# apple/ml-neuman

Hardware: NVIDIA H100
Metric: Mrays/sec @128+128 samples (higher is better)
Workload: dtype f16 operands x f32 accumulate (wgmma); f32 elsewhere

## Files before the change

neuman_b200/csrc/mlp_tc.cu:

```cuda
#include "nm_internal.cuh"
#include "nm_pe.cuh"
#include "tc_common.cuh"
#include <string.h>
#define TC_MAX_SLABS 64
struct TcPlan {
  uint32_t slab_off[TC_STEPS][6];
  uint32_t slab_bytes[TC_STEPS];
  uint32_t image_bytes;
  uint32_t lin_off[TC_MAX_SLABS + 1];
};

__host__ __device__ constexpr int tc_steps(bool v) { return v ? TC_STEPS : 9; }
__host__ __device__ constexpr int step_nkb(int s, bool v = true, bool t = false) {
  return s == 0 ? (t ? 2 : 1) : (s == 10 ? 2 : (!v && s == 8 ? 4 : (t && s == 5 ? 6 : 5)));
}
__host__ __device__ constexpr bool kb_is_bias(int s, int kb, bool v = true) {
  return kb == 4 && s != 5 && s != 9 && s >= 1 && (v ? s <= 8 : s <= 7);
}
__host__ __device__ constexpr bool kb_is_time(int s, int kb, bool t) { return t && ((s == 0 && kb == 1) || (s == 5 && kb == 5)); }
__host__ __device__ constexpr int step_N(int s, bool v = true) { return s <= 7 || (v && s == 8) ? 256 : (v && s == 9 ? 128 : 16); }
__host__ __device__ constexpr bool kb_is_dir(int s, int kb, bool v = true) { return v && s == 9 && kb == 4; }
__host__ __device__ constexpr int tc_slabs_per_tile(bool v = true, bool t = false) {
  int n = 0;
  for (int s = 0; s < tc_steps(v); ++s) n += step_nkb(s, v, t);
  return n;
}
static_assert(tc_slabs_per_tile(true, true) <= TC_MAX_SLABS && tc_slabs_per_tile(true) <= TC_MAX_SLABS, "slab table too small");

template <bool kTrain, bool kView>
struct TcCfg {
  static constexpr int THREADS = 256;
  static constexpr int NSLOT = kTrain || kView ? 4 : 6;
  static constexpr int OFF_POS = kTrain ? 4 * TC_KB_BYTES : 0;
  static constexpr int OFF_DIR = OFF_POS + TC_KB_BYTES;
  static constexpr int WG_BYTES = OFF_DIR + TC_KB_BYTES;
  static constexpr int OFF_RING = 2 * WG_BYTES;
  static constexpr int OFF_BAR = OFF_RING + NSLOT * TC_SLAB_BYTES;
  static constexpr int OFF_CONST = OFF_BAR + 16 * NSLOT;
  static constexpr int SMEM_USED = OFF_CONST + 4 * TC_CONST_FLOATS;
  static constexpr int SMEM_BYTES = SMEM_USED + 1024;
};
static_assert(TcCfg<false, false>::SMEM_BYTES <= 232448 && TcCfg<false, true>::SMEM_BYTES <= 232448 &&
              TcCfg<true, false>::SMEM_BYTES <= 232448 && TcCfg<true, true>::SMEM_BYTES <= 232448,
              "shared memory of the forward kernel exceeds 227 KB");

#define TC_CONST_ALPHA 0
#define TC_CONST_OUT 256

struct TcParams {
  const uint8_t* wimg;
  TcPlan plan;
  NmMlpInput in;
  NmPeSpec pos_pe, dir_pe;
  float* raw;
  const float* consts;
  long long n_tiles;
  int32_t* range_flag;
  int range_phase;
  __half* st_x;
  __half* st_f;
  __half* st_v;
  uint32_t* st_m;
  CUtensorMap map_x, map_f, map_v;
};

__device__ __forceinline__ void sincos_cycles(float f, float& s, float& c) {
  f = f - rintf(f);
  const float a = f * 6.283185307179586f;
  s = __sinf(a);
  c = __cosf(a);
}

__device__ __forceinline__ void encode_f16(const NmPeSpec& pe, const float x[3], uint32_t (&out)[32], int nq) {
  float ch[64];
#pragma unroll
  for (int i = 0; i < 64; ++i) ch[i] = 0.f;
// ... 94 lines not shown
    }
    const uint32_t pA = pack2<RELU>(x0, x1), pB = pack2<RELU>(y0, y1);
    if (SMEM) {
      uint8_t* blk = act + (j >> 3) * TC_KB_BYTES;
      *reinterpret_cast<uint32_t*>(blk + swz_off(rA, c)) = pA;
      *reinterpret_cast<uint32_t*>(blk + swz_off(rB, c)) = pB;
    } else {
      a[2 * j] = pA;
      a[2 * j + 1] = pB;
    }
    if (track) { track_range<RELU>(rng, pA); track_range<RELU>(rng, pB); }
    if (SIGNS) {
      const __half2 zero2 = __float2half2_rn(0.f);
      const uint32_t mA = __hgt2_mask(*reinterpret_cast<const __half2*>(&pA), zero2);
      const uint32_t mB = __hgt2_mask(*reinterpret_cast<const __half2*>(&pB), zero2);
      const int bit = 16 * ((j >> 1) & 1) + 4 * (j & 1) + q;
      wA[j >> 2] |= ((mA & 1u) << bit) | ((mA >> 16 & 1u) << (bit + 8));
      wB[j >> 2] |= ((mB & 1u) << bit) | ((mB >> 16 & 1u) << (bit + 8));
    }
  }
}

__device__ __forceinline__ void quad_or(uint32_t (&w)[8]) {
#pragma unroll
  for (int i = 0; i < 8; ++i) {
    w[i] |= __shfl_xor_sync(0xffffffffu, w[i], 1);
    w[i] |= __shfl_xor_sync(0xffffffffu, w[i], 2);
  }
}

template <bool kTrain, bool kView, bool kTime = false>
__device__ __forceinline__ void mlp_tc_body(const TcParams& P) {
  static_assert(!kTime || kView, "NeRF-T nets are view-dependent");
  using C = TcCfg<kTrain, kView>;
  constexpr int SLABS = tc_slabs_per_tile(kView, kTime);
  constexpr int STEPS = tc_steps(kView);
  constexpr int LAST = STEPS - 1;
  extern __shared__ uint8_t smem_dyn[];
  const uint32_t pad = (1024 - (smem_u32(smem_dyn) & 1023)) & 1023;
  uint8_t* smem = smem_dyn + pad;
  const uint32_t sbase = smem_u32(smem);
  const int wg = threadIdx.x >> 7, wtid = threadIdx.x & 127;
  const int lane = threadIdx.x & 31, q = lane & 3;
  const int rA = 16 * (wtid >> 5) + (lane >> 2);
  uint8_t* wbuf = smem + wg * C::WG_BYTES;
  const uint32_t wbase = sbase + wg * C::WG_BYTES;
  float* s_const = reinterpret_cast<float*>(smem + C::OFF_CONST);
  const TcRing<C::NSLOT> R{sbase + C::OFF_RING, sbase + C::OFF_BAR};

  for (int i = threadIdx.x; i < TC_CONST_FLOATS; i += C::THREADS) s_const[i] = __ldg(P.consts + i);
  const long long my_tiles = blockIdx.x < P.n_tiles ? (P.n_tiles - 1 - blockIdx.x) / gridDim.x + 1 : 0;
  const uint32_t total = (uint32_t)(my_tiles * SLABS);
  auto fill = [&](uint32_t qq) {
    const uint32_t j = qq % SLABS, off = P.plan.lin_off[j], bytes = P.plan.lin_off[j + 1] - off;
    mbar_arrive_expect_tx(R.full(qq), bytes);
    bulk_g2s(R.slot(qq), P.wimg + off, bytes, R.full(qq));
  };
  if (threadIdx.x == 0) R.init(total, fill);
  __syncthreads();

  const float4 ob = *reinterpret_cast<const float4*>(s_const + TC_CONST_OUT);
  float d[128];
  float d16[8];
  uint32_t a[64];
  uint32_t rng = 0;
  uint32_t qbase = 0;
  const long long rperiod = my_tiles < 64 ? my_tiles : 64;
  for (long long it = 0; it < my_tiles; ++it) {
    const long long tile = blockIdx.x + it * gridDim.x;
    const long long row0 = tile * 128 + wg * TC_WG_ROWS;
    const bool track = !kView || (it % rperiod) == (P.range_phase % rperiod);
    {
      const int r = wtid & 63;
      const int group = P.in.group;
      long long g0 = 0;
      uint32_t g0r = 0;
      if (group > 0) { g0 = tile * 128 / group; g0r = (uint32_t)(tile * 128 - g0 * group); }
      const uint32_t off = wg * TC_WG_ROWS + r;
      const long long g = group > 0 ? g0 + (g0r + off) / (uint32_t)group : row0 + r;
      float p[3] = {0.f, 0.f, 0.f}, v[3] = {0.f, 0.f, 0.f};
      float t = 0.f;
      if (row0 + r < P.in.n) {
        nm_fetch_sample_at<kTime ? 4 : 3>(P.in, row0 + r, g, p, v);
        if (kTime) t = nm_fetch_time(P.in, row0 + r);
      }
      if (!kTrain && it > 0) wg_sync(wg);
      uint32_t e[32];
      if (wtid < 64) {
        encode_f16(P.pos_pe, p, e, 30);
        store_row_swizzled(wbuf + C::OFF_POS, r, e, 8);
      } else if (kView) {
        encode_f16(P.dir_pe, v, e, 12);
        if (kTime) encode_time_f16(P.pos_pe, t, e);
        store_row_swizzled(wbuf + C::OFF_DIR, r, e, kTime ? 8 : 4);
      }
      if (track && (kView || wtid < 64)) { track_range<false>(rng, e[0]); track_range<false>(rng, e[1]); }
      if (kTime && track && wtid >= 64) track_range<false>(rng, e[16]);
      fence_async_smem();
      wg_sync(wg);
    }
    float alpha[2] = {0.f, 0.f};
#pragma unroll (kTrain ? 1 : STEPS)
    for (int s = 0; s < STEPS; ++s) {
      const int nkb = step_nkb(s, kView, kTime);
      const bool wide = s <= (kView ? 8 : 7), views = kView && s == 9;
      wgmma_fence();
      int kb = 0;
      auto kblock = [&](auto&& issue) {
        const uint32_t qq = qbase + kb;
        R.wait_full(qq);
        issue(gmma_desc_k(R.slot(qq)), kb == 0);
        wgmma_commit();
        if (kb > 0) { wgmma_wait<1>(); R.release(qq - 1, total, fill); }
        ++kb;
      };
      auto smem_kblock = [&](uint32_t a_addr, int k0, int k1) {
        kblock([&](uint64_t b_desc, bool first) {
          const uint64_t a_desc = gmma_desc_k(a_addr);
          for (int k = k0; k < k1; ++k) {
            const uint32_t acc = !first || k > k0;
            if (wide) wgmma_n256(d, a_desc + 2 * k, b_desc + 2 * k, acc);
            else if (views) wgmma_n128(d, a_desc + 2 * k, b_desc + 2 * k, acc);
            else wgmma_n16(d16, a_desc + 2 * k, b_desc + 2 * k, acc);
          }
        });
      };
      if (s == 0 || s == 5) smem_kblock(wbase + C::OFF_POS, 0, 4);
      if (s > 0) {
        const int nact = kView && s == LAST ? 2 : 4;
#pragma unroll
        for (int j = 0; j < 4; ++j) {
          if (j < nact) {
            if constexpr (kTrain) smem_kblock(wbase + j * TC_KB_BYTES, 0, 4);
            else kblock([&](uint64_t b_desc, bool first) {
#pragma unroll
              for (int k = 0; k < 4; ++k) {
                const uint32_t* f = a + 16 * j + 4 * k;
                const uint32_t acc = !first || k > 0;
                if (wide) wgmma_n256_rs(d, f[0], f[1], f[2], f[3], b_desc + 2 * k, acc);
                else if (views) wgmma_n128_rs(d, f[0], f[1], f[2], f[3], b_desc + 2 * k, acc);
                else wgmma_n16_rs(d16, f[0], f[1], f[2], f[3], b_desc + 2 * k, acc);
              }
            });
          }
        }
      }
      if (kb < nkb) {
        if (kb_is_bias(s, kb, kView)) smem_kblock(wbase + C::OFF_POS, 3, 4);
        else if (kb_is_dir(s, kb, kView)) smem_kblock(wbase + C::OFF_DIR, 0, 2);
        else smem_kblock(wbase + C::OFF_DIR, 2, 4);
      }
      wgmma_wait<0>();
      wgmma_fence_regs(d);
      wgmma_fence_regs(d16);
      R.release(qbase + nkb - 1, total, fill);
      qbase += nkb;
      if (s < LAST) {
        if (kTrain) {
          if (wtid == 0) tma_store_wait_read();
          wg_sync(wg);
        }
        uint32_t wA[8] = {0, 0, 0, 0, 0, 0, 0, 0}, wB[8] = {0, 0, 0, 0, 0, 0, 0, 0};
        const float* s_walpha = s_const + TC_CONST_ALPHA;
        if (s == 7) fwd_epi<256, true, kView, kTrain, kTrain>(d, a, wbuf, rA, q, s_walpha, alpha, wA, wB, track, rng);
        else if (kView && s == 8) fwd_epi<256, false, false, false, kTrain>(d, a, wbuf, rA, q, s_walpha, alpha, wA, wB, track, rng);
        else if (s == 9) fwd_epi<128, true, false, kTrain, kTrain>(d, a, wbuf, rA, q, s_walpha, alpha, wA, wB, track, rng);
        else fwd_epi<256, true, false, kTrain, kTrain>(d, a, wbuf, rA, q, s_walpha, alpha, wA, wB, track, rng);
        if (kTrain) {
          fence_async_smem();
          wg_sync(wg);
          if (wtid == 0) {
            if (!kView || s < 8) tma_store_rows(&P.map_x, wbase, 0, 4, row0, s);
            else if (s == 8) tma_store_rows(&P.map_f, wbase, 0, 4, row0, 0);
            else tma_store_rows(&P.map_v, wbase, 0, 2, row0, 0);
          }
          if (!kView || s != 8) {
            quad_or(wA);
            quad_or(wB);
            const long long iA = row0 + rA, iB = iA + 8;
            if (!kView || s < 8) {
              uint32_t* m = P.st_m + (size_t)s * P.in.n * 8;
              if (iA < P.in.n) reinterpret_cast<uint2*>(m + iA * 8)[q] = make_uint2(wA[2 * q], wA[2 * q + 1]);
              if (iB < P.in.n) reinterpret_cast<uint2*>(m + iB * 8)[q] = make_uint2(wB[2 * q], wB[2 * q + 1]);
            } else {
              uint32_t* m = P.st_m + (size_t)8 * P.in.n * 8;
              if (iA < P.in.n) m[iA * 8 + q] = wA[q];
              if (iB < P.in.n) m[iB * 8 + q] = wB[q];
            }
          }
// ... 28 lines not shown
}

template <bool kTrain>
__global__ void __launch_bounds__(TcCfg<kTrain, true>::THREADS, 1) k_mlp_tc(const __grid_constant__ TcParams P) {
  mlp_tc_body<kTrain, true>(P);
}
template <bool kTrain>
__global__ void __launch_bounds__(TcCfg<kTrain, false>::THREADS, 1) k_mlp_tc_noview(const __grid_constant__ TcParams P) {
  mlp_tc_body<kTrain, false>(P);
}
template <bool kTrain>
__global__ void __launch_bounds__(TcCfg<kTrain, true>::THREADS, 1) k_mlp_tc_nerft(const __grid_constant__ TcParams P) {
  mlp_tc_body<kTrain, true, true>(P);
}

struct PackSrc {
  const float* w[8]; const float* feat; const float* views; const float* rgb;
  const float* b[8]; const float* feat_b; const float* views_b;
  const float* out_t;
};

__device__ __forceinline__ int nerft_col(int kk, bool time) {
  if (time) {
    if (kk == 32) return 3;
    if (kk < 33 || kk > 52) return -1;
    const int k = (kk - 33) >> 1;
    return ((kk - 33) & 1) ? 11 + 8 * k : 7 + 8 * k;
  }
  if (kk < 3) return kk;
  const int i = kk - 3, k = i / 6, r = i - 6 * k;
  return r < 3 ? 4 + 8 * k + r : 8 + 8 * k + (r - 3);
}

__device__ __forceinline__ float src_weight(const PackSrc& S, int s, int n, int kb, int kk, bool view, bool time) {
  if (!view && s == 8) return n < 4 ? S.out_t[(size_t)(kb * 64 + kk) * 4 + n] : 0.f;
  if (kb_is_bias(s, kb, view)) {
    if (kk != 63) return 0.f;
    return s == 8 ? S.feat_b[n] : S.b[s][n];
  }
  if (time && (s == 0 || s == 5)) {
    const int ld = s == 0 ? NM_POS_PE_T : NM_POS_PE_T + 256;
    const float* w = S.w[s] + (size_t)n * ld;
    if (kb_is_time(s, kb, true)) {
      const int c = nerft_col(kk, true);
      return c < 0 ? 0.f : w[c];
    }
    if (kb == 0) return kk < NM_POS_PE ? w[nerft_col(kk, false)] : S.b[s][n];
    return w[NM_POS_PE_T + (kb - 1) * 64 + kk];
  }
  if (s == 0) return kk < NM_POS_PE ? S.w[0][(size_t)n * NM_POS_PE + kk] : S.b[0][n];
  if (s >= 1 && s <= 7 && s != 5) return S.w[s][(size_t)n * 256 + kb * 64 + kk];
  if (s == 5) {
    const int ld = NM_POS_PE + 256;
    if (kb == 0) return kk < NM_POS_PE ? S.w[5][(size_t)n * ld + kk] : S.b[5][n];
    return S.w[5][(size_t)n * ld + NM_POS_PE + (kb - 1) * 64 + kk];
  }
  if (s == 8) return S.feat[(size_t)n * 256 + kb * 64 + kk];
  if (s == 9) {
    const int ld = 256 + NM_DIR_PE;
    if (kb < 4) return S.views[(size_t)n * ld + kb * 64 + kk];
    return kk < NM_DIR_PE ? S.views[(size_t)n * ld + 256 + kk] : (kk == NM_DIR_PE ? S.views_b[n] : 0.f);
  }
  return n < 3 ? S.rgb[(size_t)n * 128 + kb * 64 + kk] : 0.f;
}

__global__ void k_tc_pack(PackSrc S, TcPlan plan, bool view, bool time, __half* __restrict__ out) {
  const size_t e = (size_t)blockIdx.x * blockDim.x + threadIdx.x;
  if (e * 2 >= plan.image_bytes) return;
  const uint32_t byte = (uint32_t)(e * 2);
  int s = 0, kb = 0;
  for (int ss = 0; ss < tc_steps(view); ++ss)
    for (int k = 0; k < step_nkb(ss, view, time); ++k)
      if (byte >= plan.slab_off[ss][k]) { s = ss; kb = k; }
  const uint32_t in_slab = byte - plan.slab_off[s][kb];
  const int n = in_slab >> 7;
  const int chunk_phys = (in_slab & 127) >> 4;
  const int chunk = chunk_phys ^ (n & 7);
  const int kk = chunk * 8 + ((in_slab & 15) >> 1);
  out[e] = __float2half_rn(src_weight(S, s, n, kb, kk, view, time));
}

__global__ void k_tc_consts(const float* rgb_b, const float* alpha_w, const float* alpha_b, float* __restrict__ out) {
  const int i = threadIdx.x;
  out[TC_CONST_ALPHA + i] = alpha_w[i];
  if (i < TC_CONST_FLOATS - TC_CONST_OUT) out[TC_CONST_OUT + i] = i < 3 ? rgb_b[i] : (i == 3 ? alpha_b[0] : 0.f);
}
__global__ void k_tc_consts_noview(const float* out_b, float* __restrict__ out) {
  const int i = threadIdx.x;
  out[TC_CONST_ALPHA + i] = 0.f;
  if (i < TC_CONST_FLOATS - TC_CONST_OUT) out[TC_CONST_OUT + i] = i < 4 ? out_b[i] : 0.f;
}

__global__ void k_encode_f16(NmPeSpec pe, int which, const float* __restrict__ x, long long group, long long n,
                             __half* __restrict__ out) {
  const long long i = (long long)blockIdx.x * blockDim.x + threadIdx.x;
  if (i >= n) return;
  const long long xi = group > 0 ? i / group : i;
  const float xv[3] = {x[3 * xi], x[3 * xi + 1], x[3 * xi + 2]};
  uint32_t e[32];
  encode_f16(pe, xv, e, which == 0 ? 30 : 12);
  if (which == 0) {
    e[31] |= 0x3C000000u;
    uint4* dst = reinterpret_cast<uint4*>(out + (size_t)i * 64);
#pragma unroll
    for (int j = 0; j < 8; ++j) dst[j] = make_uint4(e[4 * j], e[4 * j + 1], e[4 * j + 2], e[4 * j + 3]);
  } else {
    e[13] |= 0x3C000000u;
    uint4* dst = reinterpret_cast<uint4*>(out + (size_t)i * 32);
#pragma unroll
    for (int j = 0; j < 4; ++j) dst[j] = make_uint4(e[4 * j], e[4 * j + 1], e[4 * j + 2], e[4 * j + 3]);
  }
}
// ... 8 lines not shown
  for (int c = 0; c < 96; ++c) ch[c] = 0.f;
#pragma unroll
  for (int d = 0; d < 4; ++d) ch[d] = x[4 * xi + d];
#pragma unroll
  for (int k = 0; k < 10; ++k) {
    const float fh = __ldg(pe.table + 2 * k), fl = __ldg(pe.table + 2 * k + 1);
#pragma unroll
    for (int d = 0; d < 4; ++d) {
      const float v = ch[d];
      const float pr = v * fh;
      const float low = fmaf(v, fl, fmaf(v, fh, -pr));
      sincos_cycles((pr - rintf(pr)) + low, ch[4 + 8 * k + d], ch[8 + 8 * k + d]);
    }
  }
  ch[NM_POS_PE_T] = 1.f;
  uint4* dst = reinterpret_cast<uint4*>(out + (size_t)i * 96);
#pragma unroll
  for (int j = 0; j < 12; ++j)
    dst[j] = make_uint4(pack_f16x2(ch[8 * j], ch[8 * j + 1], false), pack_f16x2(ch[8 * j + 2], ch[8 * j + 3], false),
                        pack_f16x2(ch[8 * j + 4], ch[8 * j + 5], false), pack_f16x2(ch[8 * j + 6], ch[8 * j + 7], false));
}

int nm_tc_encode(nm_ctx* ctx, const NmNet& net, int which, const float* x, int64_t group, int64_t n, __half* out, cudaStream_t st) {
  NmPeSpec pe = which == 0 ? NmPeSpec{net.desc.pos_pe_kind, net.desc.pos_n_freqs, net.f32 + net.o_pos_cyc}
                           : NmPeSpec{net.desc.dir_pe_kind, net.desc.dir_n_freqs, net.f32 + net.o_dir_cyc};
  if (which == 0 && net.kind == NM_NET_NERFT)
    k_encode_f16_nerft<<<(unsigned)((n + 127) / 128), 128, 0, st>>>(pe, x, group, n, out);
  else
    k_encode_f16<<<(unsigned)((n + 127) / 128), 128, 0, st>>>(pe, which, x, group, n, out);
  NM_CHECK_LAUNCH(ctx);
  return NM_OK;
}

static TcPlan make_plan(bool view, bool time) {
  TcPlan p{};
  uint32_t off = 0;
  int j = 0;
  for (int s = 0; s < tc_steps(view); ++s) {
    p.slab_bytes[s] = (uint32_t)step_N(s, view) * 128u;
    for (int kb = 0; kb < step_nkb(s, view, time); ++kb) {
      p.slab_off[s][kb] = p.lin_off[j++] = off;
      off += p.slab_bytes[s];
    }
  }
  p.lin_off[j] = p.image_bytes = off;
  return p;
}

int nm_tc_pack(nm_ctx* ctx, NmNet& net, cudaStream_t st) {
  const bool view = net.kind != NM_NET_NOVIEW, time = net.kind == NM_NET_NERFT;
  TcPlan plan = make_plan(view, time);
  const size_t halfs = plan.image_bytes / 2;
  if (!net.f16 || net.f16_halfs != halfs) {
    if (net.f16) { NM_CHECK_CUDA(ctx, cudaDeviceSynchronize()); NM_CHECK_CUDA(ctx, cudaFree(net.f16)); net.f16 = nullptr; }
    NM_CHECK_CUDA(ctx, cudaMalloc(&net.f16, halfs * sizeof(__half)));
    net.f16_halfs = halfs;
  }
  if (!net.tc_bias) NM_CHECK_CUDA(ctx, cudaMalloc(&net.tc_bias, TC_CONST_FLOATS * sizeof(float)));
  const nm_nerf_desc& d = net.desc;
  PackSrc S;
  for (int l = 0; l < 8; ++l) S.w[l] = d.pts_w[l];
  S.feat = d.feature_w; S.views = d.views_w; S.rgb = d.rgb_w;
  for (int l = 0; l < 8; ++l) S.b[l] = d.pts_b[l];
  S.feat_b = d.feature_b; S.views_b = d.views_b;
  S.out_t = net.f32 + net.o_out_w;
  k_tc_pack<<<(unsigned)((halfs + 255) / 256), 256, 0, st>>>(S, plan, view, time, net.f16);
  NM_CHECK_LAUNCH(ctx);
  if (view) k_tc_consts<<<1, 256, 0, st>>>(d.rgb_b, d.alpha_w, d.alpha_b, net.tc_bias);
  else k_tc_consts_noview<<<1, 256, 0, st>>>(net.f32 + net.o_out_b, net.tc_bias);
  NM_CHECK_LAUNCH(ctx);
  return NM_OK;
}

template <bool kTrain, bool kView, bool kTime = false>
static int launch_tc(nm_ctx* ctx, const TcParams& P, cudaStream_t st) {
  void (*kernel)(const TcParams);
  if constexpr (kTime) kernel = k_mlp_tc_nerft<kTrain>;
  else kernel = kView ? k_mlp_tc<kTrain> : k_mlp_tc_noview<kTrain>;
  using C = TcCfg<kTrain, kView>;
  NM_SET_SMEM_ONCE(ctx, kernel, C::SMEM_BYTES);
  long long ctas = ctx->sm_count;
  if (P.n_tiles < ctas) ctas = P.n_tiles > 0 ? P.n_tiles : 1;
  kernel<<<(unsigned)ctas, C::THREADS, C::SMEM_BYTES, st>>>(P);
  NM_CHECK_LAUNCH(ctx);
  return NM_OK;
}

int nm_tc_forward(nm_ctx* ctx, NmNet& net, const float* pts, const float* views, const float* origins,
                  const float* dirs, const float* z, int64_t n, int32_t group, float t, float* raw, cudaStream_t st,
                  const NmTrainStash* stash) {
  if (!net.f16 || !net.tc_bias) NM_FAIL(ctx, NM_ERR_STATE, "nm_tc_forward: weights not packed");
  const bool view = net.kind != NM_NET_NOVIEW, time = net.kind == NM_NET_NERFT;
  TcParams P;
  P.wimg = reinterpret_cast<const uint8_t*>(net.f16);
  P.plan = make_plan(view, time);
  P.in = NmMlpInput{pts, views, origins, dirs, z, (long long)n, group, t};
  P.pos_pe = NmPeSpec{net.desc.pos_pe_kind, net.desc.pos_n_freqs, net.f32 + net.o_pos_cyc};
  P.dir_pe = NmPeSpec{net.desc.dir_pe_kind, net.desc.dir_n_freqs, net.f32 + net.o_dir_cyc};
  P.raw = raw;
  P.consts = net.tc_bias;
  P.n_tiles = (n + 127) / 128;
  P.range_flag = ctx->d_counter + NM_RANGE_FLAG_WORD;
  P.range_phase = (int)(ctx->range_seq++ % 64);
  P.st_x = stash ? stash->x : nullptr; P.st_f = stash ? stash->f : nullptr; P.st_v = stash ? stash->v : nullptr;
  P.st_m = stash ? stash->m : nullptr;
  memset(&P.map_x, 0, 3 * sizeof(CUtensorMap));
  if (stash) {
    if (n >= (int64_t)0x7fff0000) NM_FAIL(ctx, NM_ERR_INVALID, "nm_mlp_forward_train: n too large for one call");
    if (tc_make_store_map(&P.map_x, stash->x, 8, (uint64_t)n, 256) ||
        (view && (tc_make_store_map(&P.map_f, stash->f, 1, (uint64_t)n, 256) || tc_make_store_map(&P.map_v, stash->v, 1, (uint64_t)n, 128))))
      NM_FAIL(ctx, NM_ERR_CUDA, "nm_mlp_forward_train: cuTensorMapEncodeTiled failed");
  }
  if (time) return stash ? launch_tc<true, true, true>(ctx, P, st) : launch_tc<false, true, true>(ctx, P, st);
  if (!view) return stash ? launch_tc<true, false>(ctx, P, st) : launch_tc<false, false>(ctx, P, st);
  return stash ? launch_tc<true, true>(ctx, P, st) : launch_tc<false, true>(ctx, P, st);
}
```

neuman_b200/csrc/tc_common.cuh:

```cuda
#pragma once
#include "nm_internal.cuh"

#define TC_STEPS 11
#define TC_CONST_FLOATS 272
#define TC_WG_ROWS 64
#define TC_KB_BYTES (TC_WG_ROWS * 128)
#define TC_SLAB_BYTES 32768

__device__ __forceinline__ uint32_t smem_u32(const void* p) { return (uint32_t)__cvta_generic_to_shared(p); }

__device__ __forceinline__ void mbar_init(uint32_t bar, uint32_t count) {
  asm volatile("mbarrier.init.shared::cta.b64 [%0], %1;" ::"r"(bar), "r"(count) : "memory");
}
__device__ __forceinline__ void mbar_wait(uint32_t bar, uint32_t parity) {
  asm volatile(
      "{\n\t"
      ".reg .pred P1;\n\t"
      "WAIT_LOOP:\n\t"
      "mbarrier.try_wait.parity.shared::cta.b64 P1, [%0], %1;\n\t"
      "@P1 bra DONE;\n\t"
      "bra WAIT_LOOP;\n\t"
      "DONE:\n\t"
      "}" ::"r"(bar), "r"(parity) : "memory");
}
__device__ __forceinline__ void st_shared_u32(uint32_t addr, uint32_t v) {
  asm volatile("st.shared.u32 [%0], %1;" ::"r"(addr), "r"(v) : "memory");
}
__device__ __forceinline__ uint32_t atom_add_acq_rel_cta(uint32_t addr, uint32_t v) {
  uint32_t old;
  asm volatile("atom.acq_rel.cta.shared::cta.add.u32 %0, [%1], %2;" : "=r"(old) : "r"(addr), "r"(v) : "memory");
  return old;
}
__device__ __forceinline__ void mbar_arrive_expect_tx(uint32_t bar, uint32_t bytes) {
  asm volatile("mbarrier.arrive.expect_tx.shared::cta.b64 _, [%0], %1;" ::"r"(bar), "r"(bytes) : "memory");
}
__device__ __forceinline__ void bulk_g2s(uint32_t dst, const void* src, uint32_t bytes, uint32_t bar) {
  asm volatile("cp.async.bulk.shared::cluster.global.mbarrier::complete_tx::bytes [%0], [%1], %2, [%3];" ::"r"(dst),
               "l"(src), "r"(bytes), "r"(bar) : "memory");
}
__device__ __forceinline__ void fence_async_smem() { asm volatile("fence.proxy.async.shared::cta;" ::: "memory"); }
__device__ __forceinline__ void fence_mbar_init() { asm volatile("fence.mbarrier_init.release.cluster;" ::: "memory"); }
__device__ __forceinline__ void wg_sync(int wg) { asm volatile("bar.sync %0, 128;" ::"r"(wg + 1) : "memory"); }

__device__ __forceinline__ uint64_t gmma_desc_k(uint32_t saddr) {
  return (uint64_t)((saddr & 0x3FFFFu) >> 4) | ((uint64_t)1 << 16) | ((uint64_t)(1024 >> 4) << 32) | ((uint64_t)1 << 62);
}
__device__ __forceinline__ uint64_t gmma_desc_mn(uint32_t saddr, uint32_t lbo) {
  return (uint64_t)((saddr & 0x3FFFFu) >> 4) | ((uint64_t)(lbo >> 4) << 16) | ((uint64_t)(1024 >> 4) << 32) |
         ((uint64_t)1 << 62);
}

__device__ __forceinline__ void wgmma_fence() { asm volatile("wgmma.fence.sync.aligned;" ::: "memory"); }
__device__ __forceinline__ void wgmma_commit() { asm volatile("wgmma.commit_group.sync.aligned;" ::: "memory"); }
template <int N>
__device__ __forceinline__ void wgmma_wait() { asm volatile("wgmma.wait_group.sync.aligned %0;" ::"n"(N) : "memory"); }
template <int R>
__device__ __forceinline__ void wgmma_fence_regs(float (&d)[R]) {
#pragma unroll
  for (int i = 0; i < R; ++i) asm volatile("" : "+f"(d[i])::"memory");
}

__device__ __forceinline__ void wgmma_n256(float (&d)[128], uint64_t a_desc, uint64_t b_desc, uint32_t accum) {
  asm volatile(
      "{\n\t.reg .pred p;\n\tsetp.ne.b32 p, %130, 0;\n\t"
      "wgmma.mma_async.sync.aligned.m64n256k16.f32.f16.f16 "
      "{%0, %1, %2, %3, %4, %5, %6, %7, %8, %9, %10, %11, %12, %13, %14, %15, %16, %17, %18, %19, %20, %21, %22, %23, %24, %25, %26, %27, %28, %29, %30, %31, %32, %33, %34, %35, %36, %37, %38, %39, %40, %41, %42, %43, %44, %45, %46, %47, %48, %49, %50, %51, %52, %53, %54, %55, %56, %57, %58, %59, %60, %61, %62, %63, %64, %65, %66, %67, %68, %69, %70, %71, %72, %73, %74, %75, %76, %77, %78, %79, %80, %81, %82, %83, %84, %85, %86, %87, %88, %89, %90, %91, %92, %93, %94, %95, %96, %97, %98, %99, %100, %101, %102, %103, %104, %105, %106, %107, %108, %109, %110, %111, %112, %113, %114, %115, %116, %117, %118, %119, %120, %121, %122, %123, %124, %125, %126, %127}, "
      "%128, %129, p, 1, 1, 0, 0;\n\t}"
      : "+f"(d[0]), "+f"(d[1]), "+f"(d[2]), "+f"(d[3]), "+f"(d[4]), "+f"(d[5]), "+f"(d[6]), "+f"(d[7]), "+f"(d[8]), "+f"(d[9]), "+f"(d[10]), "+f"(d[11]), "+f"(d[12]), "+f"(d[13]), "+f"(d[14]), "+f"(d[15]), "+f"(d[16]), "+f"(d[17]), "+f"(d[18]), "+f"(d[19]), "+f"(d[20]), "+f"(d[21]), "+f"(d[22]), "+f"(d[23]), "+f"(d[24]), "+f"(d[25]), "+f"(d[26]), "+f"(d[27]), "+f"(d[28]), "+f"(d[29]), "+f"(d[30]), "+f"(d[31]), "+f"(d[32]), "+f"(d[33]), "+f"(d[34]), "+f"(d[35]), "+f"(d[36]), "+f"(d[37]), "+f"(d[38]), "+f"(d[39]), "+f"(d[40]), "+f"(d[41]), "+f"(d[42]), "+f"(d[43]), "+f"(d[44]), "+f"(d[45]), "+f"(d[46]), "+f"(d[47]), "+f"(d[48]), "+f"(d[49]), "+f"(d[50]), "+f"(d[51]), "+f"(d[52]), "+f"(d[53]), "+f"(d[54]), "+f"(d[55]), "+f"(d[56]), "+f"(d[57]), "+f"(d[58]), "+f"(d[59]), "+f"(d[60]), "+f"(d[61]), "+f"(d[62]), "+f"(d[63]), "+f"(d[64]), "+f"(d[65]), "+f"(d[66]), "+f"(d[67]), "+f"(d[68]), "+f"(d[69]), "+f"(d[70]), "+f"(d[71]), "+f"(d[72]), "+f"(d[73]), "+f"(d[74]), "+f"(d[75]), "+f"(d[76]), "+f"(d[77]), "+f"(d[78]), "+f"(d[79]), "+f"(d[80]), "+f"(d[81]), "+f"(d[82]), "+f"(d[83]), "+f"(d[84]), "+f"(d[85]), "+f"(d[86]), "+f"(d[87]), "+f"(d[88]), "+f"(d[89]), "+f"(d[90]), "+f"(d[91]), "+f"(d[92]), "+f"(d[93]), "+f"(d[94]), "+f"(d[95]), "+f"(d[96]), "+f"(d[97]), "+f"(d[98]), "+f"(d[99]), "+f"(d[100]), "+f"(d[101]), "+f"(d[102]), "+f"(d[103]), "+f"(d[104]), "+f"(d[105]), "+f"(d[106]), "+f"(d[107]), "+f"(d[108]), "+f"(d[109]), "+f"(d[110]), "+f"(d[111]), "+f"(d[112]), "+f"(d[113]), "+f"(d[114]), "+f"(d[115]), "+f"(d[116]), "+f"(d[117]), "+f"(d[118]), "+f"(d[119]), "+f"(d[120]), "+f"(d[121]), "+f"(d[122]), "+f"(d[123]), "+f"(d[124]), "+f"(d[125]), "+f"(d[126]), "+f"(d[127])
      : "l"(a_desc), "l"(b_desc), "r"(accum));
}
__device__ __forceinline__ void wgmma_n128(float (&d)[128], uint64_t a_desc, uint64_t b_desc, uint32_t accum) {
  asm volatile(
      "{\n\t.reg .pred p;\n\tsetp.ne.b32 p, %66, 0;\n\t"
      "wgmma.mma_async.sync.aligned.m64n128k16.f32.f16.f16 "
      "{%0, %1, %2, %3, %4, %5, %6, %7, %8, %9, %10, %11, %12, %13, %14, %15, %16, %17, %18, %19, %20, %21, %22, %23, %24, %25, %26, %27, %28, %29, %30, %31, %32, %33, %34, %35, %36, %37, %38, %39, %40, %41, %42, %43, %44, %45, %46, %47, %48, %49, %50, %51, %52, %53, %54, %55, %56, %57, %58, %59, %60, %61, %62, %63}, "
      "%64, %65, p, 1, 1, 0, 0;\n\t}"
      : "+f"(d[0]), "+f"(d[1]), "+f"(d[2]), "+f"(d[3]), "+f"(d[4]), "+f"(d[5]), "+f"(d[6]), "+f"(d[7]), "+f"(d[8]), "+f"(d[9]), "+f"(d[10]), "+f"(d[11]), "+f"(d[12]), "+f"(d[13]), "+f"(d[14]), "+f"(d[15]), "+f"(d[16]), "+f"(d[17]), "+f"(d[18]), "+f"(d[19]), "+f"(d[20]), "+f"(d[21]), "+f"(d[22]), "+f"(d[23]), "+f"(d[24]), "+f"(d[25]), "+f"(d[26]), "+f"(d[27]), "+f"(d[28]), "+f"(d[29]), "+f"(d[30]), "+f"(d[31]), "+f"(d[32]), "+f"(d[33]), "+f"(d[34]), "+f"(d[35]), "+f"(d[36]), "+f"(d[37]), "+f"(d[38]), "+f"(d[39]), "+f"(d[40]), "+f"(d[41]), "+f"(d[42]), "+f"(d[43]), "+f"(d[44]), "+f"(d[45]), "+f"(d[46]), "+f"(d[47]), "+f"(d[48]), "+f"(d[49]), "+f"(d[50]), "+f"(d[51]), "+f"(d[52]), "+f"(d[53]), "+f"(d[54]), "+f"(d[55]), "+f"(d[56]), "+f"(d[57]), "+f"(d[58]), "+f"(d[59]), "+f"(d[60]), "+f"(d[61]), "+f"(d[62]), "+f"(d[63])
      : "l"(a_desc), "l"(b_desc), "r"(accum));
// ... 135 lines not shown
```

neuman_b200/csrc/warp.cu:

```cuda
#include <cub/device/device_radix_sort.cuh>
#include <float.h>
#include <math.h>

#include "nm_internal.cuh"
#include "train_common_kernels.cuh"

struct BvhView {
  int n;
  const float4* lo;
  const float4* hi;
  const int2* children;
  const int32_t* leaf_face;
  const float* tri9;
};

__device__ __forceinline__ uint32_t expand_bits10(uint32_t v) {
  v = (v * 0x00010001u) & 0xFF0000FFu;
  v = (v * 0x00000101u) & 0x0F00F00Fu;
  v = (v * 0x00000011u) & 0xC30C30C3u;
  v = (v * 0x00000005u) & 0x49249249u;
  return v;
}

__device__ __forceinline__ int f2ord(float f) { const int k = __float_as_int(f); return k >= 0 ? k : k ^ 0x7fffffff; }
// ... 103 lines not shown
  return {a.y * b.z - a.z * b.y, a.z * b.x - a.x * b.z, a.x * b.y - a.y * b.x};
}

template <typename T>
__device__ __forceinline__ V3<T> closest_on_tri(V3<T> p, V3<T> a, V3<T> b, V3<T> c) {
  V3<T> ab = sub(b, a), ac = sub(c, a), ap = sub(p, a);
  T d1 = dot(ab, ap), d2 = dot(ac, ap);
  if (d1 <= 0 && d2 <= 0) return a;
  V3<T> bp = sub(p, b);
  T d3 = dot(ab, bp), d4 = dot(ac, bp);
  if (d3 >= 0 && d4 <= d3) return b;
  T vc = d1 * d4 - d3 * d2;
  if (vc <= 0 && d1 >= 0 && d3 <= 0) return madd(a, ab, d1 / (d1 - d3));
  V3<T> cp = sub(p, c);
  T d5 = dot(ab, cp), d6 = dot(ac, cp);
  if (d6 >= 0 && d5 <= d6) return c;
  T vb = d5 * d2 - d1 * d6;
  if (vb <= 0 && d2 >= 0 && d6 <= 0) return madd(a, ac, d2 / (d2 - d6));
  T va = d3 * d6 - d5 * d4;
  if (va <= 0 && (d4 - d3) >= 0 && (d5 - d6) >= 0) return madd(b, sub(c, b), (d4 - d3) / ((d4 - d3) + (d5 - d6)));
  T den = T(1) / (va + vb + vc);
  return madd(madd(a, ab, vb * den), ac, vc * den);
}

__device__ __forceinline__ float box_d2(const BvhView& B, int node, V3<float> p) {
  const float4 l = __ldg(B.lo + node), h = __ldg(B.hi + node);
  float dx = fmaxf(fmaxf(l.x - p.x, p.x - h.x), 0.f), dy = fmaxf(fmaxf(l.y - p.y, p.y - h.y), 0.f),
        dz = fmaxf(fmaxf(l.z - p.z, p.z - h.z), 0.f);
  return dx * dx + dy * dy + dz * dz;
}

__device__ __forceinline__ int bvh_nearest_face(const BvhView& B, V3<float> p, int* stack) {
  float best = FLT_MAX;
  int best_f = 0x7fffffff;
  int sp = 0;
  int node = (B.n > 1) ? 0 : B.n - 1;
  while (true) {
    if (node >= B.n - 1) {
      const int f = __ldg(B.leaf_face + (node - (B.n - 1)));
      const float* t = B.tri9 + 9 * (size_t)f;
      V3<float> a{__ldg(t), __ldg(t + 1), __ldg(t + 2)}, b{__ldg(t + 3), __ldg(t + 4), __ldg(t + 5)},
          c{__ldg(t + 6), __ldg(t + 7), __ldg(t + 8)};
      V3<float> e = sub(closest_on_tri<float>(p, a, b, c), p);
      const float d2 = dot(e, e);
      if (d2 < best || (d2 == best && f < best_f)) { best = d2; best_f = f; }
      node = -1;
    } else {
      const int2 ch = __ldg(B.children + node);
      const float dl = box_d2(B, ch.x, p), dr = box_d2(B, ch.y, p);
      const float lim = best * 1.00001f;
      const bool needL = __any_sync(0xffffffffu, dl <= lim), needR = __any_sync(0xffffffffu, dr <= lim);
      const bool left_first = __popc(__ballot_sync(0xffffffffu, dl <= dr)) >= 16;
      if (needL && needR) {
        if (sp < 64) { if ((threadIdx.x & 31) == 0) stack[sp] = left_first ? ch.y : ch.x; ++sp; }
        node = left_first ? ch.x : ch.y;
      } else {
        node = needL ? ch.x : (needR ? ch.y : -1);
      }
    }
    if (node < 0) {
      bool found = false;
      while (sp > 0) {
        --sp;
        __syncwarp();
        const int cand = stack[sp];
        if (__any_sync(0xffffffffu, box_d2(B, cand, p) <= best * 1.00001f)) { node = cand; found = true; break; }
      }
      if (!found) break;
    }
  }
  return best_f;
}

__global__ void __launch_bounds__(128) k_warp_nearest(BvhView B, const float* __restrict__ pts, long long R, int S, int lg_rays,
                                                       int32_t* __restrict__ face_out) {
  const long long w = (long long)blockIdx.x * 4 + (threadIdx.x >> 5);
  const int lane = threadIdx.x & 31;
  long long i;
// ... 348 lines not shown
```

Baseline: 1.468.

## Keep bias, dir, time and output weight slabs resident in smem, stream only dense slabs

The inference MLP kernel now loads a small tail of weights once per CTA into shared memory. The tail holds the bias, direction, time and output slabs, packed at reduced row widths (32/64 bytes) with matching swizzle descriptors. Only the dense K-blocks are streamed through the TMA ring each tile, and bias addition becomes a register-sourced one-hot wgmma. The change cuts per-tile bulk copies and ring waits, but adds smem pressure (the ring shrinks from 6 to 5 slots for the view net) and a new packing layout. The warp BVH nearest-face search also gains a double-precision tie refinement, which adds cost there.

```diff
diff --git a/neuman_b200/csrc/mlp_tc.cu b/neuman_b200/csrc/mlp_tc.cu
--- a/neuman_b200/csrc/mlp_tc.cu
+++ b/neuman_b200/csrc/mlp_tc.cu
@@ -2,12 +2,13 @@
 #include "nm_pe.cuh"
 #include "tc_common.cuh"
 #include <string.h>
-#define TC_MAX_SLABS 64
+#define TC_MAX_FILLS 64
 struct TcPlan {
-  uint32_t slab_off[TC_STEPS][6];
-  uint32_t slab_bytes[TC_STEPS];
+  uint32_t kb_off[TC_STEPS][6];
+  uint32_t fill_off[TC_MAX_FILLS];
+  uint32_t fill_bytes[TC_MAX_FILLS];
+  uint32_t tail_off;
   uint32_t image_bytes;
-  uint32_t lin_off[TC_MAX_SLABS + 1];
 };
 
 __host__ __device__ constexpr int tc_steps(bool v) { return v ? TC_STEPS : 9; }
@@ -18,30 +19,55 @@
   return kb == 4 && s != 5 && s != 9 && s >= 1 && (v ? s <= 8 : s <= 7);
 }
 __host__ __device__ constexpr bool kb_is_time(int s, int kb, bool t) { return t && ((s == 0 && kb == 1) || (s == 5 && kb == 5)); }
+__host__ __device__ constexpr int bias_col(int s) { return s <= 4 ? s - 1 : s - 2; }
 __host__ __device__ constexpr int step_N(int s, bool v = true) { return s <= 7 || (v && s == 8) ? 256 : (v && s == 9 ? 128 : 16); }
 __host__ __device__ constexpr bool kb_is_dir(int s, int kb, bool v = true) { return v && s == 9 && kb == 4; }
-__host__ __device__ constexpr int tc_slabs_per_tile(bool v = true, bool t = false) {
+
+#define TC_TAIL_BIAS 0u
+#define TC_TAIL_DIR 8192u
+__host__ __device__ constexpr uint32_t tc_tail_time(int s) { return s == 0 ? 16384u : 32768u; }
+__host__ __device__ constexpr uint32_t tc_tail_out(bool v, bool t) { return !v ? 8192u : (t ? 49152u : 16384u); }
+__host__ __device__ constexpr uint32_t tc_tail_bytes(bool v, bool t) { return tc_tail_out(v, t) + (v ? 2u : 4u) * 2048u; }
+__host__ __device__ constexpr int kb_tail(int s, int kb, bool v, bool t) {
+  return kb_is_bias(s, kb, v) ? (int)TC_TAIL_BIAS
+       : kb_is_dir(s, kb, v) ? (int)TC_TAIL_DIR
+       : kb_is_time(s, kb, t) ? (int)tc_tail_time(s)
+       : s == tc_steps(v) - 1 ? (int)(tc_tail_out(v, t) + 2048u * kb) : -1;
+}
+__host__ __device__ constexpr int kb_row(int s, int kb, bool v, bool t) {
+  return kb_is_bias(s, kb, v) ? 32 : (kb_is_dir(s, kb, v) || kb_is_time(s, kb, t) ? 64 : 128);
+}
+__host__ __device__ constexpr uint32_t kb_bytes(int s, int kb, bool v, bool t) { return (uint32_t)(step_N(s, v) * kb_row(s, kb, v, t)); }
+__host__ __device__ constexpr int tc_fills_per_tile(bool v, bool t, bool train) {
   int n = 0;
-  for (int s = 0; s < tc_steps(v); ++s) n += step_nkb(s, v, t);
+  for (int s = 0; s < tc_steps(v); ++s)
+    for (int kb = 0; kb < step_nkb(s, v, t); ++kb) n += train || kb_tail(s, kb, v, t) < 0;
   return n;
 }
-static_assert(tc_slabs_per_tile(true, true) <= TC_MAX_SLABS && tc_slabs_per_tile(true) <= TC_MAX_SLABS, "slab table too small");
-
-template <bool kTrain, bool kView>
+static_assert(tc_fills_per_tile(true, true, true) <= TC_MAX_FILLS && tc_fills_per_tile(true, false, true) <= TC_MAX_FILLS,
+              "fill table too small");
+static_assert(tc_fills_per_tile(true, false, false) == 38 && tc_fills_per_tile(true, true, false) == 38 &&
+              tc_fills_per_tile(false, false, false) == 30, "streamed slabs per tile");
+
+template <bool kTrain, bool kView, bool kTime = false>
 struct TcCfg {
   static constexpr int THREADS = 256;
-  static constexpr int NSLOT = kTrain || kView ? 4 : 6;
+  static constexpr int NSLOT = kTrain || kTime ? 4 : (kView ? 5 : 6);
   static constexpr int OFF_POS = kTrain ? 4 * TC_KB_BYTES : 0;
   static constexpr int OFF_DIR = OFF_POS + TC_KB_BYTES;
-  static constexpr int WG_BYTES = OFF_DIR + TC_KB_BYTES;
+  static constexpr int WG_BYTES = OFF_DIR + (kView ? TC_KB_BYTES : 0);
   static constexpr int OFF_RING = 2 * WG_BYTES;
-  static constexpr int OFF_BAR = OFF_RING + NSLOT * TC_SLAB_BYTES;
-  static constexpr int OFF_CONST = OFF_BAR + 16 * NSLOT;
+  static constexpr int OFF_TAIL = OFF_RING + NSLOT * TC_SLAB_BYTES;
+  static constexpr int TAIL_BYTES = kTrain ? 0 : (int)tc_tail_bytes(kView, kTime);
+  static constexpr int OFF_BAR = OFF_TAIL + TAIL_BYTES;
+  static constexpr int OFF_TAIL_BAR = OFF_BAR + 16 * NSLOT;
+  static constexpr int OFF_CONST = OFF_TAIL_BAR + 16;
   static constexpr int SMEM_USED = OFF_CONST + 4 * TC_CONST_FLOATS;
   static constexpr int SMEM_BYTES = SMEM_USED + 1024;
 };
 static_assert(TcCfg<false, false>::SMEM_BYTES <= 232448 && TcCfg<false, true>::SMEM_BYTES <= 232448 &&
-              TcCfg<true, false>::SMEM_BYTES <= 232448 && TcCfg<true, true>::SMEM_BYTES <= 232448,
+              TcCfg<false, true, true>::SMEM_BYTES <= 232448 && TcCfg<true, false>::SMEM_BYTES <= 232448 &&
+              TcCfg<true, true>::SMEM_BYTES <= 232448 && TcCfg<true, true, true>::SMEM_BYTES <= 232448,
               "shared memory of the forward kernel exceeds 227 KB");
 
 #define TC_CONST_ALPHA 0
@@ -202,8 +228,8 @@
 template <bool kTrain, bool kView, bool kTime = false>
 __device__ __forceinline__ void mlp_tc_body(const TcParams& P) {
   static_assert(!kTime || kView, "NeRF-T nets are view-dependent");
-  using C = TcCfg<kTrain, kView>;
-  constexpr int SLABS = tc_slabs_per_tile(kView, kTime);
+  using C = TcCfg<kTrain, kView, kTime>;
+  constexpr int FILLS = tc_fills_per_tile(kView, kTime, kTrain);
   constexpr int STEPS = tc_steps(kView);
   constexpr int LAST = STEPS - 1;
   extern __shared__ uint8_t smem_dyn[];
@@ -217,17 +243,26 @@
   const uint32_t wbase = sbase + wg * C::WG_BYTES;
   float* s_const = reinterpret_cast<float*>(smem + C::OFF_CONST);
   const TcRing<C::NSLOT> R{sbase + C::OFF_RING, sbase + C::OFF_BAR};
+  const uint32_t tail = sbase + C::OFF_TAIL, tail_bar = sbase + C::OFF_TAIL_BAR;
 
   for (int i = threadIdx.x; i < TC_CONST_FLOATS; i += C::THREADS) s_const[i] = __ldg(P.consts + i);
   const long long my_tiles = blockIdx.x < P.n_tiles ? (P.n_tiles - 1 - blockIdx.x) / gridDim.x + 1 : 0;
-  const uint32_t total = (uint32_t)(my_tiles * SLABS);
+  const uint32_t total = (uint32_t)(my_tiles * FILLS);
   auto fill = [&](uint32_t qq) {
-    const uint32_t j = qq % SLABS, off = P.plan.lin_off[j], bytes = P.plan.lin_off[j + 1] - off;
+    const uint32_t j = qq % FILLS, off = P.plan.fill_off[j], bytes = P.plan.fill_bytes[j];
     mbar_arrive_expect_tx(R.full(qq), bytes);
     bulk_g2s(R.slot(qq), P.wimg + off, bytes, R.full(qq));
   };
-  if (threadIdx.x == 0) R.init(total, fill);
+  if (threadIdx.x == 0) {
+    if (!kTrain) mbar_init(tail_bar, 1);
+    R.init(total, fill);
+    if (!kTrain) {
+      mbar_arrive_expect_tx(tail_bar, C::TAIL_BYTES);
+      bulk_g2s(tail, P.wimg + P.plan.tail_off, C::TAIL_BYTES, tail_bar);
+    }
+  }
   __syncthreads();
+  if (!kTrain) mbar_wait(tail_bar, 0);
 
   const float4 ob = *reinterpret_cast<const float4*>(s_const + TC_CONST_OUT);
   float d[128];
@@ -274,24 +309,30 @@
     for (int s = 0; s < STEPS; ++s) {
       const int nkb = step_nkb(s, kView, kTime);
       const bool wide = s <= (kView ? 8 : 7), views = kView && s == 9;
+      const int bc = bias_col(s);
+      const uint32_t one_hot = q == (bc >> 1) ? ((bc & 1) ? 0x3C000000u : 0x3C00u) : 0u;
       wgmma_fence();
       int kb = 0;
-      auto kblock = [&](auto&& issue) {
-        const uint32_t qq = qbase + kb;
-        R.wait_full(qq);
-        issue(gmma_desc_k(R.slot(qq)), kb == 0);
+      uint32_t qq = qbase;
+      bool held = false;
+      auto kblock = [&](bool resident, uint32_t b_tail, auto&& issue) {
+        resident = resident && !kTrain;
+        if (!resident) R.wait_full(qq);
+        issue(resident ? tail + b_tail : R.slot(qq), kb == 0);
         wgmma_commit();
-        if (kb > 0) { wgmma_wait<1>(); R.release(qq - 1, total, fill); }
+        if (kb > 0) { wgmma_wait<1>(); if (held) R.release(qq - 1, total, fill); }
+        held = !resident;
+        qq += !resident;
         ++kb;
       };
-      auto smem_kblock = [&](uint32_t a_addr, int k0, int k1) {
-        kblock([&](uint64_t b_desc, bool first) {
-          const uint64_t a_desc = gmma_desc_k(a_addr);
+      auto smem_kblock = [&](uint32_t a_addr, int k0, int k1, bool narrow = false, int b_tail = -1) {
+        kblock(b_tail >= 0, (uint32_t)b_tail, [&](uint32_t b, bool first) {
+          const uint64_t a_desc = gmma_desc_k(a_addr), b_desc = narrow ? gmma_desc_k<64>(b) : gmma_desc_k(b);
           for (int k = k0; k < k1; ++k) {
             const uint32_t acc = !first || k > k0;
-            if (wide) wgmma_n256(d, a_desc + 2 * k, b_desc + 2 * k, acc);
-            else if (views) wgmma_n128(d, a_desc + 2 * k, b_desc + 2 * k, acc);
-            else wgmma_n16(d16, a_desc + 2 * k, b_desc + 2 * k, acc);
+            if (wide) wgmma_n256(d, a_desc + 2 * k, b_desc + 2 * (k - k0), acc);
+            else if (views) wgmma_n128(d, a_desc + 2 * k, b_desc + 2 * (k - k0), acc);
+            else wgmma_n16(d16, a_desc + 2 * k, b_desc + 2 * (k - k0), acc);
           }
         });
       };
@@ -301,8 +342,10 @@
 #pragma unroll
         for (int j = 0; j < 4; ++j) {
           if (j < nact) {
-            if constexpr (kTrain) smem_kblock(wbase + j * TC_KB_BYTES, 0, 4);
-            else kblock([&](uint64_t b_desc, bool first) {
+            const int out = s == LAST ? kb_tail(s, j, kView, kTime) : -1;
+            if constexpr (kTrain) smem_kblock(wbase + j * TC_KB_BYTES, 0, 4, false, out);
+            else kblock(out >= 0, (uint32_t)out, [&](uint32_t b, bool first) {
+              const uint64_t b_desc = gmma_desc_k(b);
 #pragma unroll
               for (int k = 0; k < 4; ++k) {
                 const uint32_t* f = a + 16 * j + 4 * k;
@@ -316,15 +359,16 @@
         }
       }
       if (kb < nkb) {
-        if (kb_is_bias(s, kb, kView)) smem_kblock(wbase + C::OFF_POS, 3, 4);
-        else if (kb_is_dir(s, kb, kView)) smem_kblock(wbase + C::OFF_DIR, 0, 2);
-        else smem_kblock(wbase + C::OFF_DIR, 2, 4);
+        if (kb_is_bias(s, kb, kView))
+          kblock(true, TC_TAIL_BIAS, [&](uint32_t b, bool) { wgmma_n256_rs(d, one_hot, one_hot, 0u, 0u, gmma_desc_k<32>(b), 1); });
+        else if (kb_is_dir(s, kb, kView)) smem_kblock(wbase + C::OFF_DIR, 0, 2, true, TC_TAIL_DIR);
+        else if (kb_is_time(s, kb, kTime)) smem_kblock(wbase + C::OFF_DIR, 2, 4, true, tc_tail_time(s));
       }
       wgmma_wait<0>();
       wgmma_fence_regs(d);
       wgmma_fence_regs(d16);
-      R.release(qbase + nkb - 1, total, fill);
-      qbase += nkb;
+      if (held) R.release(qq - 1, total, fill);
+      qbase = qq;
       if (s < LAST) {
         if (kTrain) {
           if (wtid == 0) tma_store_wait_read();
@@ -419,12 +463,14 @@
   return r < 3 ? 4 + 8 * k + r : 8 + 8 * k + (r - 3);
 }
 
+__device__ __forceinline__ float bias_weight(const PackSrc& S, int n, int c, bool view) {
+  if (c >= (view ? 7 : 6)) return 0.f;
+  const int s = c < 4 ? c + 1 : c + 2;
+  return s == 8 ? S.feat_b[n] : S.b[s][n];
+}
+
 __device__ __forceinline__ float src_weight(const PackSrc& S, int s, int n, int kb, int kk, bool view, bool time) {
   if (!view && s == 8) return n < 4 ? S.out_t[(size_t)(kb * 64 + kk) * 4 + n] : 0.f;
-  if (kb_is_bias(s, kb, view)) {
-    if (kk != 63) return 0.f;
-    return s == 8 ? S.feat_b[n] : S.b[s][n];
-  }
   if (time && (s == 0 || s == 5)) {
     const int ld = s == 0 ? NM_POS_PE_T : NM_POS_PE_T + 256;
     const float* w = S.w[s] + (size_t)n * ld;
@@ -458,13 +504,15 @@
   int s = 0, kb = 0;
   for (int ss = 0; ss < tc_steps(view); ++ss)
     for (int k = 0; k < step_nkb(ss, view, time); ++k)
-      if (byte >= plan.slab_off[ss][k]) { s = ss; kb = k; }
-  const uint32_t in_slab = byte - plan.slab_off[s][kb];
-  const int n = in_slab >> 7;
-  const int chunk_phys = (in_slab & 127) >> 4;
-  const int chunk = chunk_phys ^ (n & 7);
-  const int kk = chunk * 8 + ((in_slab & 15) >> 1);
-  out[e] = __float2half_rn(src_weight(S, s, n, kb, kk, view, time));
+      if (byte >= plan.kb_off[ss][k] && byte < plan.kb_off[ss][k] + kb_bytes(ss, k, view, time)) { s = ss; kb = k; }
+  const int row = kb_row(s, kb, view, time);
+  const uint32_t in_slab = byte - plan.kb_off[s][kb];
+  const int n = in_slab / row;
+  const int chunk = ((in_slab % row) >> 4) ^ ((in_slab >> 7) & (row / 16 - 1));
+  const int c = chunk * 8 + ((in_slab & 15) >> 1);
+  const float w = kb_is_bias(s, kb, view) ? bias_weight(S, n, c, view)
+                : src_weight(S, s, n, kb, kb_is_time(s, kb, time) ? 32 + c : c, view, time);
+  out[e] = __float2half_rn(w);
 }
 
 __global__ void k_tc_consts(const float* rgb_b, const float* alpha_w, const float* alpha_b, float* __restrict__ out) {
@@ -539,24 +587,33 @@
   return NM_OK;
 }
 
-static TcPlan make_plan(bool view, bool time) {
+static TcPlan make_plan(bool view, bool time, bool train) {
   TcPlan p{};
   uint32_t off = 0;
+  for (int s = 0; s < tc_steps(view); ++s)
+    for (int kb = 0; kb < step_nkb(s, view, time); ++kb)
+      if (kb_tail(s, kb, view, time) < 0) {
+        p.kb_off[s][kb] = off;
+        off += kb_bytes(s, kb, view, time);
+      }
+  p.tail_off = off;
+  p.image_bytes = off + tc_tail_bytes(view, time);
   int j = 0;
-  for (int s = 0; s < tc_steps(view); ++s) {
-    p.slab_bytes[s] = (uint32_t)step_N(s, view) * 128u;
+  for (int s = 0; s < tc_steps(view); ++s)
     for (int kb = 0; kb < step_nkb(s, view, time); ++kb) {
-      p.slab_off[s][kb] = p.lin_off[j++] = off;
-      off += p.slab_bytes[s];
-    }
-  }
-  p.lin_off[j] = p.image_bytes = off;
+      const int t = kb_tail(s, kb, view, time);
+      if (t >= 0) p.kb_off[s][kb] = p.tail_off + (uint32_t)t;
+      if (train || t < 0) {
+        p.fill_off[j] = p.kb_off[s][kb];
+        p.fill_bytes[j++] = kb_bytes(s, kb, view, time);
+      }
+    }
   return p;
 }
 
 int nm_tc_pack(nm_ctx* ctx, NmNet& net, cudaStream_t st) {
   const bool view = net.kind != NM_NET_NOVIEW, time = net.kind == NM_NET_NERFT;
-  TcPlan plan = make_plan(view, time);
+  TcPlan plan = make_plan(view, time, false);
   const size_t halfs = plan.image_bytes / 2;
   if (!net.f16 || net.f16_halfs != halfs) {
     if (net.f16) { NM_CHECK_CUDA(ctx, cudaDeviceSynchronize()); NM_CHECK_CUDA(ctx, cudaFree(net.f16)); net.f16 = nullptr; }
@@ -584,7 +641,7 @@
   void (*kernel)(const TcParams);
   if constexpr (kTime) kernel = k_mlp_tc_nerft<kTrain>;
   else kernel = kView ? k_mlp_tc<kTrain> : k_mlp_tc_noview<kTrain>;
-  using C = TcCfg<kTrain, kView>;
+  using C = TcCfg<kTrain, kView, kTime>;
   NM_SET_SMEM_ONCE(ctx, kernel, C::SMEM_BYTES);
   long long ctas = ctx->sm_count;
   if (P.n_tiles < ctas) ctas = P.n_tiles > 0 ? P.n_tiles : 1;
@@ -600,7 +657,7 @@
   const bool view = net.kind != NM_NET_NOVIEW, time = net.kind == NM_NET_NERFT;
   TcParams P;
   P.wimg = reinterpret_cast<const uint8_t*>(net.f16);
-  P.plan = make_plan(view, time);
+  P.plan = make_plan(view, time, stash != nullptr);
   P.in = NmMlpInput{pts, views, origins, dirs, z, (long long)n, group, t};
   P.pos_pe = NmPeSpec{net.desc.pos_pe_kind, net.desc.pos_n_freqs, net.f32 + net.o_pos_cyc};
   P.dir_pe = NmPeSpec{net.desc.dir_pe_kind, net.desc.dir_n_freqs, net.f32 + net.o_dir_cyc};
diff --git a/neuman_b200/csrc/tc_common.cuh b/neuman_b200/csrc/tc_common.cuh
--- a/neuman_b200/csrc/tc_common.cuh
+++ b/neuman_b200/csrc/tc_common.cuh
@@ -42,8 +42,11 @@
 __device__ __forceinline__ void fence_mbar_init() { asm volatile("fence.mbarrier_init.release.cluster;" ::: "memory"); }
 __device__ __forceinline__ void wg_sync(int wg) { asm volatile("bar.sync %0, 128;" ::"r"(wg + 1) : "memory"); }
 
+template <int ROW = 128>
 __device__ __forceinline__ uint64_t gmma_desc_k(uint32_t saddr) {
-  return (uint64_t)((saddr & 0x3FFFFu) >> 4) | ((uint64_t)1 << 16) | ((uint64_t)(1024 >> 4) << 32) | ((uint64_t)1 << 62);
+  static_assert(ROW == 128 || ROW == 64 || ROW == 32, "GMMA K-major swizzle widths");
+  constexpr uint64_t layout = ROW == 128 ? 1 : (ROW == 64 ? 2 : 3);
+  return (uint64_t)((saddr & 0x3FFFFu) >> 4) | ((uint64_t)1 << 16) | ((uint64_t)(8 * ROW >> 4) << 32) | (layout << 62);
 }
 __device__ __forceinline__ uint64_t gmma_desc_mn(uint32_t saddr, uint32_t lbo) {
   return (uint64_t)((saddr & 0x3FFFFu) >> 4) | ((uint64_t)(lbo >> 4) << 16) | ((uint64_t)(1024 >> 4) << 32) |
diff --git a/neuman_b200/csrc/warp.cu b/neuman_b200/csrc/warp.cu
--- a/neuman_b200/csrc/warp.cu
+++ b/neuman_b200/csrc/warp.cu
@@ -159,6 +159,7 @@
 
 __device__ __forceinline__ int bvh_nearest_face(const BvhView& B, V3<float> p, int* stack) {
   float best = FLT_MAX;
+  double best64 = DBL_MAX;
   int best_f = 0x7fffffff;
   int sp = 0;
   int node = (B.n > 1) ? 0 : B.n - 1;
@@ -170,7 +171,13 @@
           c{__ldg(t + 6), __ldg(t + 7), __ldg(t + 8)};
       V3<float> e = sub(closest_on_tri<float>(p, a, b, c), p);
       const float d2 = dot(e, e);
-      if (d2 < best || (d2 == best && f < best_f)) { best = d2; best_f = f; }
+      if (d2 <= best * 1.00001f) {
+        const V3<double> pd{p.x, p.y, p.z}, ad{a.x, a.y, a.z}, bd{b.x, b.y, b.z}, cd{c.x, c.y, c.z};
+        const V3<double> ed = sub(closest_on_tri<double>(pd, ad, bd, cd), pd);
+        const double dd = dot(ed, ed);
+        if (dd < best64 || (dd == best64 && f < best_f)) { best64 = dd; best_f = f; }
+        best = fminf(best, d2);
+      }
       node = -1;
     } else {
       const int2 ch = __ldg(B.children + node);
```

After: 1.540 (median of 6 runs). 4.9% higher.
